# fujii-team/Henbun

Measured on AMD Instinct MI355X. Metric: elbo_samples_per_sec, higher is better.
Workload: dtype f32; 1 GPU; cfg2 SVGP ELBO step: 1-D UnitRBF, N=1e6, M=512 inducing, minibatch 8192 per GPU, diag Normal q(u), diagonal residual, Adam lr 1e-3; global_batch=8192, per_gpu_batch=8192, parallelism=dp1, N=1000000, M=512, dp_exchange=none, dp_ranks=1, contraction=native, tri_pack=False

## Files before the change

### henbun_amd/_lib.py

```python
from __future__ import annotations

import ctypes
import os
from ctypes import c_char_p, c_double, c_int, c_long, c_uint64, c_void_p

_HERE = os.path.dirname(os.path.abspath(__file__))
LIB_PATH = os.path.join(_HERE, "libhenbun_hip.so")


class HipBackendError(RuntimeError):
    """A libhenbun_hip.so entry point returned a non-zero status."""


P, L, I, D, U64 = c_void_p, c_long, c_int, c_double, c_uint64

_SIGS = {
    "hb_version": [],
    "hb_debug_set": [c_char_p, L],
    "hb_debug_clear": [],
    "hb_cholesky_inverse_ws_elems": [L, L, I],
    "hb_cholesky_persistent_shape": [L, L, I],
    "hb_mlp2_sample_supported": [L, L, L, L, L, I],
    "hb_mlp2_sample_ws_elems": [L, L, L],
    "hb_mlp2_sample_fwd_f32": [P, P, P, P, P, I, P, P, L, P, P, P, P, L, L, L, P, P],
    "hb_mlp2_sample_bwd_f32": [P, P, P, P, I, P, P, P, P, P, P, P, P, P, L, L, L, P, P],
    "hb_gram_cholesky_inverse_f32": [I, P, L, P, L, L, L, D, P, P, L, L, P, P, P, I, P],
    "hb_last_error_string": [],
    "hb_device_info": [P, I, P],
    "hb_graph_begin_capture": [P],
    "hb_graph_end_capture": [P, P],
    "hb_graph_launch": [P, P],
    "hb_graph_destroy": [P],
    "hb_rng_init": [P, L, U64, U64, P],
    "hb_rng_randint": [P, L, P, L, L, L, P],
    "hb_sgp_ws_elems": [L, L, L, L, L],
    "hb_sgp_strip_path": [L, L, L, L, L, I],
    "hb_sgp_head_units": [L, L, L, L, L, I, I, I, L],
    "hb_sgp_rider_supported": [L, L, L, L, L, I, I, I, L],
    "hb_sgp_predict_ws_elems": [L, L, L, L, L, I, I, I],
    "hb_sgp_predict_cov_ws_elems": [L, L, L, L, I, I],
    "hb_sgp_stats_ws_elems": [L, L, L, L, I],
    "hb_sgp_select_ws_elems": [L, L, L, I],
    "hb_gram_matvec_chunk": [],
    "hb_gram_matvec_ws_elems": [L, L, L, I],
    "hb_gram_bilinear_grad_ws_elems": [L, L],
    "hb_sgp_kgrad_ws_elems": [L, L, L, L],
    "hb_sgp_wstats_ws_elems": [L, L, L, I],
    "hb_lik_sites_ws_elems": [L],
    "hb_matmul_gauss_units": [L, L, L],
    "hb_matmul_gram_vjp_ok": [L, L, L, L],
    "hb_matmul_gram_vjp_ws_elems": [L, L, L],
    "hb_matmul_gram_vjp_f32": [P, P, P, L, L, L, L, L, L, L, L, L, I, I, P, L, P, L, L, L, P, P, P, P, P],
    "hb_fullrank_one_launch_shape": [L, L],
    "hb_matmul_gauss_f32": [P, L, P, L, P, P, P, P, D, P, P, P, L, L, L, L, P],
    "hb_sgp_rider_begin": [],
    "hb_sgp_rider_pending": [],
    "hb_sgp_rider_flush": [P],
    "hb_sgp_fwd_gauss_f32": [I, I, P, L, P, P, L, P, P, I, P, P, P, L, P, P, P, P, P, L, L, L, L, L, P, P, P, P, D, P, P, P, L, P],
    "hb_ewise_prog_image_bytes": [],
# ... 142 lines not shown
```

### henbun_amd/csrc/sgp.hip

```cpp
#include "common.cuh"
#include "sgp_strip.cuh"
#include "chain.cuh"
#include "chol_persist.cuh"
#include <type_traits>
#include "gemm_tile.cuh"
#include "rng_pairs.cuh"
#include "../../include/henbun_hip.h"

#define SGP_BM 64
#define SGP_BN 128

extern "C" int hb_matmul_f32(const float*, const float*, float*, long, long, long, long, long, long, long, long, long,
                             long, int, int, double, double, const float*, long, int, int, float*, long, void*);
extern "C" int hb_matmul_f64(const double*, const double*, double*, long, long, long, long, long, long, long, long,
                             long, long, int, int, double, double, const double*, long, int, int, double*, long,
                             void*);

template <typename T>
struct SgpArgs {
  const T* x;
  long sx;
  const T* z;
  const T* ell;
  long dl;
// ... 1762 lines not shown
template <typename T>
struct SgpBwdArgs {
  const T* W;
  const T* u;
  const T* A;
  const T* fbar;
  const T* eps;
  const T* v;
  T* Kbar;
  long n, M, P;
  int mode;
  long efast;
  const T* x;
  long sx;
  const T* z;
  const T* ell;
  long dl, d;
  const T* WTf;
  const void* WT3;
  long plane3;
  T* part;
  const T* Af;
  T* Kf;
};

template <typename T>
struct SgpRawB {
  T a, u;
};
template <typename T>
struct SgpRawB4 {
  typedef T VT __attribute__((ext_vector_type(16 / sizeof(T))));
  VT a;
  T u;
};

template <typename T, bool FAST>
__global__ void __launch_bounds__(256) sgp_kbar_kernel(SgpBwdArgs<T> a) {
  typedef TileGemm<T, SGP_BM, SGP_BN, 16, 2, 2> G;
  __shared__ __attribute__((aligned(16))) T lds[G::LDS_ELEMS];
  long e;
  int bx;
  sgp_block(a.efast, e, bx);
  const T* W = a.W + e * a.M * a.M;
  const T* u = a.u + e * a.P * a.M;
  const T* A = a.A + e * a.M * a.n;
// ... 137 lines not shown
  SgpStageZ<D, SGP_STRIP_THREADS> zst;
  SgpStageU<SGP_STRIP_THREADS> ust;
  zst.request(z, M, tid);
  ust.request(a.u + e * a.P * a.M, P, M, tid);
  if (tid < SGP_SN) {
    const int cc = col0 + tid;
    const bool ok = cc < n;
    const int cj = ok ? cc : n - 1;
    cjs[tid] = ok ? sgp_resid_coef<float>(a.eps ? a.eps + e * a.n : nullptr, a.v + e * a.n, fbar, a.n, a.P, a.mode, cj) : 0.f;
#pragma unroll
    for (int p = 0; p < 4; ++p) fbs[p][tid] = (ok && p < P) ? fbar[(long)p * n + cj] : 0.f;
#pragma unroll
    for (int dd = 0; dd < D; ++dd) xss[tid * D + dd] = x[cj * D + dd];
  }
  zst.store(zs, M, tid);
  ust.store(us, P, M, tid);
  __syncthreads();

  if (a.Af) {
    const int nTp = M / 32;
    const long fplane = (long)a.plane3 / a.M * 32 * nS;
    for (int t = w; t < nTp; t += SGP_STRIP_THREADS / 64) {
      float avals[16];
      if (BF3) {
        const __bf16* blk = reinterpret_cast<const __bf16*>(a.Af) + ((((long)e * nTp + t) * nS + bx) << 10) + 8 * lane;
        B8 pl[3][2];
#pragma unroll
        for (int p = 0; p < 3; ++p)
#pragma unroll
          for (int q = 0; q < 2; ++q) pl[p][q] = *reinterpret_cast<const B8*>(blk + p * fplane + 512 * q);
#pragma unroll
        for (int q = 0; q < 2; ++q)
#pragma unroll
          for (int j = 0; j < 8; ++j) avals[8 * q + j] = ((float)pl[2][q][j] + (float)pl[1][q][j]) + (float)pl[0][q][j];
      } else {
        const float* blk = a.Af + ((((long)e * nTp + t) * nS + bx) << 10) + 4 * lane;
        V4 av[4];
#pragma unroll
        for (int v = 0; v < 4; ++v) av[v] = *reinterpret_cast<const V4*>(blk + 256 * v);
#pragma unroll
        for (int v = 0; v < 4; ++v)
#pragma unroll
          for (int s2 = 0; s2 < 4; ++s2) avals[4 * v + s2] = av[v][s2];
      }
      const int k = 32 * t + li;
      float uk[4], usum[4] = {0.f, 0.f, 0.f, 0.f};
#pragma unroll
      for (int p = 0; p < 4; ++p) uk[p] = p < P ? us[p][k] : 0.f;
#pragma unroll
      for (int v = 0; v < 4; ++v) {
        const V4 cj4 = *reinterpret_cast<const V4*>(&cjs[16 * h + 4 * v]);
        V4 fb4[4];
#pragma unroll
        for (int p = 0; p < 4; ++p) fb4[p] = *reinterpret_cast<const V4*>(&fbs[p][16 * h + 4 * v]);
#pragma unroll
        for (int s2 = 0; s2 < 4; ++s2) {
          const int c = 16 * h + 4 * v + s2;
          const float aval = avals[4 * v + s2];
          float val = aval * cj4[s2];
#pragma unroll
          for (int p = 0; p < 4; ++p)
            if (p < P) {
              val += uk[p] * fb4[p][s2];
              usum[p] += fb4[p][s2] * aval;
            }
          if (BF3) {
            const __bf16 b0 = (__bf16)val;
            const float r1 = val - (float)b0;
            const __bf16 b1 = (__bf16)r1;
            K3[0][c][k] = b0, K3[1][c][k] = b1, K3[2][c][k] = (__bf16)(r1 - (float)b1);
          } else {
            Ks[c][k] = val;
          }
        }
      }
#pragma unroll
      for (int p = 0; p < 4; ++p)
        if (p < P) {
          const float tsum = usum[p] + __shfl_xor(usum[p], 32);
          if (h == 0) part[(long)(2 * D + p) * M + k] = tsum;
        }
    }
  } else {
    constexpr int G = BF3 ? 8 : 4;
    const int c = tid & 31, kq = tid >> 5;
    const bool cok = col0 + c < n;
    const int cc = cok ? col0 + c : n - 1;
    const float cj = cjs[c];
    float fb[4];
#pragma unroll
    for (int p = 0; p < 4; ++p) fb[p] = fbs[p][c];
    constexpr int NG = SGP_SM_MAX / (16 * G);
    float av[NG][G];
#pragma unroll
    for (int it = 0; it < NG; ++it)
#pragma unroll
      for (int i = 0; i < G; ++i) {
// ... 65 lines not shown
    float kb[16];
    sgp_acc_t_rows(acc, kb);
    if (col0 + SGP_SN > n) {
#pragma unroll
      for (int i = 0; i < 16; ++i)
        if (col0 + 16 * h + i >= n) kb[i] = 0.f;
    }
    if (a.Kbar) {
      float* kp = Kbar + (long)(32 * tile + li) * n + col0 + 16 * h;
      if ((n & 3) == 0 && col0 + SGP_SN <= n) {
#pragma unroll
        for (int v = 0; v < 4; ++v) {
          V4 q;
#pragma unroll
          for (int s2 = 0; s2 < 4; ++s2) q[s2] = kb[4 * v + s2];
          *reinterpret_cast<V4*>(kp + 4 * v) = q;
        }
      } else {
#pragma unroll
        for (int i = 0; i < 16; ++i)
          if (col0 + 16 * h + i < n) kp[i] = kb[i];
      }
    }
    if (a.Kf && !BF3) sgp_store_frag_rows(a.Kf, kb, e, nT, nS, tile, bx, col0, n, lane);
    if (BF3 && a.Kf)
      sgp_store_frag3_row(reinterpret_cast<__bf16*>(a.Kf), (long)a.plane3 / a.M * 32 * nS, kb, e, nT, nS, tile, bx, lane);
    const int row = 32 * tile + li;
    float zr[D], zacc[D], lacc[D];
#pragma unroll
    for (int dd = 0; dd < D; ++dd) zr[dd] = zs[row * D + dd], zacc[dd] = 0.f, lacc[dd] = 0.f;
#pragma unroll
    for (int i = 0; i < 16; ++i) {
      const int c = 16 * h + i;
      float tt[D], r2 = 0.f;
#pragma unroll
      for (int dd = 0; dd < D; ++dd) {
        tt[dd] = (zr[dd] - xss[c * D + dd]) * col.sc[dd];
        r2 += tt[dd] * tt[dd];
      }
      const float gk = kb[i] * hb_exp2_neg<float>(r2);
#pragma unroll
      for (int dd = 0; dd < D; ++dd) {
        zacc[dd] -= gk * tt[dd];
        lacc[dd] += gk * tt[dd] * tt[dd];
      }
    }
#pragma unroll
// ... 369 lines not shown
__device__ __forceinline__ void sgp_lbar_finish_body(const T* __restrict__ slabs, int S, long E, long M, T* __restrict__ Lbar,
                                                     long vblock, long nvblocks) {
  const long total = E * M * M;
  const long stride = nvblocks * blockDim.x;
  for (long t = vblock * blockDim.x + threadIdx.x; t < total; t += stride) {
    const long rem = t % (M * M);
    const long r = rem / M, c = rem - r * M;
    T acc = T(0);
    if (c <= r) {
      T a0 = T(0), a1 = T(0), a2 = T(0), a3 = T(0);
      int s = 0;
      for (; s + 4 <= S; s += 4) {
        const T v0 = slabs[(long)s * total + t], v1 = slabs[(long)(s + 1) * total + t];
        const T v2 = slabs[(long)(s + 2) * total + t], v3 = slabs[(long)(s + 3) * total + t];
        a0 += v0, a1 += v1, a2 += v2, a3 += v3;
      }
      for (; s < S; ++s) a0 += slabs[(long)s * total + t];
      acc = -((a0 + a1) + (a2 + a3));
    }
    Lbar[t] = acc;
  }
}
template <typename T>
__global__ void __launch_bounds__(256) sgp_lbar_finish_kernel(const T* __restrict__ slabs, int S, long E, long M,
                                                              T* __restrict__ Lbar) {
  sgp_lbar_finish_body<T>(slabs, S, E, M, Lbar, blockIdx.x, gridDim.x);
}

template <typename T>
__device__ __forceinline__ void sgp_strip_finish_body(const T* __restrict__ part, int nS, long M, long d, long dl, long P,
                                                      T* __restrict__ zbar, T* __restrict__ ellbar, T* __restrict__ ubar,
                                                      int bx, int q, long e, T (*red)[64], T* smem) {
  const int nq = (int)(2 * d + P);
  part += e * nS * (long)nq * M;
  if (q >= (int)d && q < 2 * (int)d) {
    if (bx != 0) return;
    T acc = T(0);
    for (int s = threadIdx.x; s < nS; s += 256) acc += part[((long)s * nq + q) * M];
    acc = block_sum(acc, smem);
    if (dl == 1) {
      if (q != (int)d) return;
      T tot = acc;
      for (int qq = (int)d + 1; qq < 2 * (int)d; ++qq) {
        T a2 = T(0);
        for (int s = threadIdx.x; s < nS; s += 256) a2 += part[((long)s * nq + qq) * M];
        tot += block_sum(a2, smem);
// ... 23 lines not shown
  red[sg][ml] = acc;
  __syncthreads();
  if (sg == 0 && m < M) {
    const T tot = (red[0][ml] + red[1][ml]) + (red[2][ml] + red[3][ml]);
    if (q < (int)d)
      zbar[(e * M + m) * d + q] = tot;
    else
      ubar[(e * P + (q - 2 * d)) * M + m] = tot;
  }
}
template <typename T>
__global__ void __launch_bounds__(256) sgp_strip_finish_kernel(const T* __restrict__ part, int nS, long M, long d, long dl,
                                                               long P, T* __restrict__ zbar, T* __restrict__ ellbar,
                                                               T* __restrict__ ubar) {
  __shared__ T red[4][64];
  __shared__ T smem[16];
  sgp_strip_finish_body<T>(part, nS, M, d, dl, P, zbar, ellbar, ubar, (int)blockIdx.x, (int)blockIdx.y, (long)blockIdx.z, red, smem);
}
template <typename T>
__global__ void __launch_bounds__(256) sgp_bwd_finish_kernel(const T* __restrict__ part, int nS, long M, long d, long dl,
                                                             long P, T* __restrict__ zbar, T* __restrict__ ellbar,
                                                             T* __restrict__ ubar, int nb_strip, int nbx,
                                                             const T* __restrict__ slabs, int S, long E,
                                                             T* __restrict__ Lbar) {
  __shared__ T red[4][64];
  __shared__ T smem[16];
  if ((int)blockIdx.x < nb_strip) {
    const int nq = (int)(2 * d + P);
    const int vb = blockIdx.x;
    sgp_strip_finish_body<T>(part, nS, M, d, dl, P, zbar, ellbar, ubar, vb % nbx, (vb / nbx) % nq, (long)(vb / (nbx * nq)), red,
                             smem);
  } else {
    sgp_lbar_finish_body<T>(slabs, S, E, M, Lbar, (long)blockIdx.x - nb_strip, (long)gridDim.x - nb_strip);
  }
}

template <typename T>
__global__ void __launch_bounds__(256) sgp_rowgrad_kernel(const T* __restrict__ x, long sx, const T* __restrict__ z,
                                                          const T* __restrict__ ell, long dl,
                                                          const T* __restrict__ Kbar, const T* __restrict__ A,
                                                          const T* __restrict__ fbar, T* __restrict__ zbar,
                                                          T* __restrict__ ellpart, T* __restrict__ ubar, long n,
                                                          long M, long d, long P) {
  __shared__ T smem[16];
  const long e = blockIdx.y, m = blockIdx.x;
  x += e * sx;
  z += (e * M + m) * d;
  ell += e * dl;
  Kbar += (e * M + m) * n;
  A += (e * M + m) * n;
  fbar += e * P * n;
  const long npass_p = (P + 3) / 4, npass_q = (d + SGP_DREG - 1) / SGP_DREG;
  const long npass = npass_p > npass_q ? npass_p : npass_q;
  for (long pass = 0; pass < npass; ++pass) {
// ... 248 lines not shown
        HB_LAUNCH_CHECK();
        *S_out = (int)S2;
        return 0;
      }
    }
  }
  dim3 grid((unsigned)(pairs * S * E), 1, 1);
  if (prec == HB_PREC_BF16X3)
    hipLaunchKernelGGL(sgp_lbar_frag_kernel<true>, grid, dim3(256), 0, stream, Kf, Af, slabs, (int)M, (int)nS, (int)S, E,
                       (int)pairs);
  else
    hipLaunchKernelGGL(sgp_lbar_frag_kernel<false>, grid, dim3(256), 0, stream, Kf, Af, slabs, (int)M, (int)nS, (int)S, E,
                       (int)pairs);
  HB_LAUNCH_CHECK();
  *S_out = (int)S;
  return 0;
}
static int sgp_lbar_frag_launch(const double*, const double*, double*, long, long, long, long, int, int*, hipStream_t) { return -1; }

template <typename T>
static int sgp_bwd(int kind, int mode, const T* x, long sx, const T* z, const T* ell, long dl, const T* W,
                   const T* Wfrag, int prec, const T* u, const T* eps, const T* A, const T* A_frag, const T* v,
                   const T* fbar, T* Kbar, T* Kbar_frag, T* Lbar, T* ubar, T* zbar, T* ellbar, T* xbar, long E, long n,
                   long M, long d, long P, T* ws, hipStream_t stream) {
  HB_REQUIRE(prec == HB_PREC_NATIVE || prec == HB_PREC_BF16X3, "hb_sgp_bwd: unknown precision %d", prec);
  HB_REQUIRE(kind == HB_KERN_RBF, "hb_sgp_bwd: only the UnitRBF kernel is fused (kind=%d)", kind);
  HB_REQUIRE(mode == HB_SGP_NEGLECTED || mode == HB_SGP_DIAGONAL, "hb_sgp_bwd: unknown mode %d", mode);
  HB_REQUIRE(E >= 0 && n >= 0 && M >= 0 && d >= 1 && P >= 0, "hb_sgp_bwd: bad extents");
  HB_REQUIRE(dl == 1 || dl == d, "hb_sgp_bwd: lengthscales must have 1 or d entries");
  HB_REQUIRE(x && z && ell && W && u && (A || A_frag) && v && fbar && (Kbar || Kbar_frag) && Lbar && ubar && zbar && ellbar && ws,
             "hb_sgp_bwd: NULL pointer");
  HB_REQUIRE((A_frag != nullptr) == (Kbar_frag != nullptr), "hb_sgp_bwd: A_frag and Kbar_frag go together");
  HB_REQUIRE(mode == HB_SGP_NEGLECTED || eps, "hb_sgp_bwd: eps required for the diagonal mode");
  HB_REQUIRE(E <= 65535, "hb_sgp_bwd: too many experts");
  HB_REQUIRE(M * n < 2147483647L && M * M < 2147483647L && n * d < 2147483647L, "hb_sgp_bwd: matrix too large for 32-bit indexing");
  if (E * M == 0) return 0;
  T* ellpart = ws + E * n;
  T* mmws = ellpart + E * M * d;
  const long mmws_elems = 32 * E * M * M;
  const long nS = hb_cdiv(n, SGP_SN);
  const bool strip = sizeof(T) == 4 && Wfrag && !xbar && hb_sgp_strip_path(E, n, M, d, P, prec) &&
                     nS * (2 * d + P) * M * E <= mmws_elems;
  HB_REQUIRE(!A_frag || strip, "hb_sgp_bwd: fragment-major A / Kbar need the column-strip form (see hb_sgp_strip_path)");
  HB_REQUIRE(strip || (A && Kbar), "hb_sgp_bwd: row-major A and Kbar required outside the column-strip form");
  HB_REQUIRE(prec == HB_PREC_NATIVE || strip, "hb_sgp_bwd: bf16x3 needs the column-strip form (fp32, Wfrag, M %% 32 == 0, M <= %d, "
             "d <= %d, P <= 4, no xbar)", SGP_SM_MAX, SGP_DREG);
  if (strip) {
    SgpBwdArgs<T> a;
    a.W = W; a.u = u; a.A = A; a.fbar = fbar; a.eps = eps; a.v = v; a.Kbar = Kbar;
    a.n = n; a.M = M; a.P = P; a.mode = mode;
    a.x = x; a.sx = sx; a.z = z; a.ell = ell; a.dl = dl; a.d = d;
    a.WTf = Wfrag + E * M * M;
    a.WT3 = prec == HB_PREC_BF16X3 ? (const void*)(reinterpret_cast<const unsigned short*>(Wfrag + 2 * E * M * M) + 3 * E * M * M)
                                   : nullptr;
    a.plane3 = E * M * M;
    a.part = mmws;
    a.Af = A_frag; a.Kf = Kbar_frag;
    if (A_frag) a.Kbar = nullptr;
    int rc = sgp_bwd_strip_launch(a, E, nS, stream);
    if (rc) return rc;
    if (A_frag) {
      const long npart = ((nS * (2 * d + P) * M * E + 63) / 64) * 64;
      const long slab_cap = (mmws_elems - npart) / (E * M * M);
      HB_REQUIRE(slab_cap >= 1, "hb_sgp_bwd: workspace too small for the Lbar slabs");
      int S = 0;
      rc = sgp_lbar_frag_launch(Kbar_frag, A_frag, mmws + npart, slab_cap > 32 ? 32 : slab_cap, E, M, nS, prec, &S, stream);
      if (rc) return rc;
      const int nbx = (int)hb_cdiv(M, 64), nb_strip = nbx * (int)(2 * d + P) * (int)E;
      hipLaunchKernelGGL(sgp_bwd_finish_kernel<T>, dim3((unsigned)(nb_strip + hb_stream_grid(E * M * M, 256))), dim3(256), 0, stream,
                         mmws, (int)nS, M, d, dl, P, zbar, ellbar, ubar, nb_strip, nbx, mmws + npart, S, E, Lbar);
      HB_LAUNCH_CHECK();
      return 0;
    }
    hipLaunchKernelGGL(sgp_strip_finish_kernel<T>, dim3((unsigned)hb_cdiv(M, 64), (unsigned)(2 * d + P), (unsigned)E), dim3(256), 0,
                       stream, mmws, (int)nS, M, d, dl, P, zbar, ellbar, ubar);
    HB_LAUNCH_CHECK();
    int rc2 = sgp_matmul(Kbar, A, Lbar, E, M, M, n, n, n, M, M * n, M * n, M * M, 0, 1, -1.0, HB_MM_TRIL_OUT, mmws, mmws_elems,
                         (void*)stream);
    return rc2;
  }
  if (n > 0) {
    SgpBwdArgs<T> a;
    a.W = W; a.u = u; a.A = A; a.fbar = fbar; a.eps = eps; a.v = v; a.Kbar = Kbar;
    a.n = n; a.M = M; a.P = P; a.mode = mode;
    a.x = nullptr; a.sx = 0; a.z = nullptr; a.ell = nullptr; a.dl = 0; a.d = d; a.WTf = nullptr; a.WT3 = nullptr;
    a.plane3 = 0; a.part = nullptr; a.Af = nullptr; a.Kf = nullptr;
    const int nRB = hb_cdiv(M, SGP_BM);
    dim3 grid = sgp_grid(hb_cdiv(n, SGP_BN), sgp_grid_y(E, n, nRB), E, a.efast);
    constexpr long VECH = 16 / sizeof(T);
    const bool vec = P == 1 && M % 16 == 0 && n % VECH == 0 && ((uintptr_t)W % 16 == 0) && ((uintptr_t)A % 16 == 0);
    if (vec)
      hipLaunchKernelGGL((sgp_kbar_kernel<T, true>), grid, dim3(256), 0, stream, a);
    else
      hipLaunchKernelGGL((sgp_kbar_kernel<T, false>), grid, dim3(256), 0, stream, a);
    HB_LAUNCH_CHECK();
  }
  {
    constexpr long VECR = 16 / sizeof(T);
    const bool rvec = d <= SGP_DREG && P <= 4 && n > 0 && n % VECR == 0 && ((uintptr_t)A % 16 == 0) &&
                      ((uintptr_t)Kbar % 16 == 0) && ((uintptr_t)fbar % 16 == 0) && ((uintptr_t)x % 16 == 0) &&
                      (sx * (long)sizeof(T)) % 16 == 0;
    dim3 rgrid((unsigned)M, (unsigned)E);
#define HB_SGP_ROWGRAD(D_)                                                                                           \
  hipLaunchKernelGGL((sgp_rowgrad_vec_kernel<T, D_>), rgrid, dim3(256), 0, stream, x, sx, z, ell, dl, Kbar, A, fbar, \
                     zbar, ellpart, ubar, n, M, P)
    if (rvec && d == 1)
      HB_SGP_ROWGRAD(1);
    else if (rvec && d == 2)
      HB_SGP_ROWGRAD(2);
// ... 21 lines not shown
    if (rc) return rc;
  } else {
    HB_HIP(hb_zero_async(Lbar, sizeof(T) * E * M * M, stream));
  }
  return 0;
}

extern "C" int hb_sgp_bwd_f32(int kind, int mode, const float* x, long sx, const float* z, const float* ell, long dl,
                              const float* W, const float* Wfrag, int prec, const float* u, const float* eps,
                              const float* A, const float* A_frag, const float* v, const float* fbar, float* Kbar,
                              float* Kbar_frag, float* Lbar, float* ubar, float* zbar, float* ellbar, float* xbar, long E,
                              long n, long M, long d, long P, float* ws, void* stream) {
  return sgp_bwd<float>(kind, mode, x, sx, z, ell, dl, W, Wfrag, prec, u, eps, A, A_frag, v, fbar, Kbar, Kbar_frag, Lbar,
                        ubar, zbar, ellbar, xbar, E, n, M, d, P, ws, (hipStream_t)stream);
}
extern "C" int hb_sgp_bwd_f64(int kind, int mode, const double* x, long sx, const double* z, const double* ell,
                              long dl, const double* W, const double* Wfrag, int prec, const double* u, const double* eps,
                              const double* A, const double* A_frag, const double* v, const double* fbar, double* Kbar,
                              double* Kbar_frag, double* Lbar, double* ubar, double* zbar, double* ellbar, double* xbar,
                              long E, long n, long M, long d, long P, double* ws, void* stream) {
  return sgp_bwd<double>(kind, mode, x, sx, z, ell, dl, W, Wfrag, prec, u, eps, A, A_frag, v, fbar, Kbar, Kbar_frag, Lbar,
                         ubar, zbar, ellbar, xbar, E, n, M, d, P, ws, (hipStream_t)stream);
}
```

### henbun_amd/graph.py

```python
from __future__ import annotations

import itertools
import math
from typing import Dict, List, Optional, Sequence, Tuple

import numpy as np

from ._lib import HipBackendError as _HipBackendError

_uid = itertools.count()



class Node:
    __slots__ = ("op", "inputs", "attrs", "outputs", "id")

    def __init__(self, op, inputs, attrs, out_shapes):
        self.op = op
        self.inputs = tuple(inputs)
        self.attrs = attrs
        self.id = next(_uid)
        self.outputs = [Tensor(self, i, tuple(int(d) for d in s)) for i, s in enumerate(out_shapes)]


# ... 805 lines not shown
    axis = axis % nd
    return concat([expand_dims(v, axis) for v in vals], axis)


def matmul(a, b, transpose_a=False, transpose_b=False, bias=None, act="none") -> Tensor:
    a, b = as_tensor(a), as_tensor(b)
    if len(a.shape) < 2 or len(b.shape) < 2:
        raise ValueError("matmul needs rank >= 2 operands")
    m, k = (a.shape[-1], a.shape[-2]) if transpose_a else (a.shape[-2], a.shape[-1])
    k2, n = (b.shape[-1], b.shape[-2]) if transpose_b else (b.shape[-2], b.shape[-1])
    if k != k2:
        raise ValueError("matmul inner dimensions differ: %s x %s" % (a.shape, b.shape))
    la, lb = a.shape[:-2], b.shape[:-2]
    if la and lb and la != lb:
        raise ValueError("matmul batch dimensions differ: %s vs %s" % (la, lb))
    lead = la if la else lb
    ins = (a, b) if bias is None else (a, b, as_tensor(bias))
    return make("matmul", ins, {"ta": bool(transpose_a), "tb": bool(transpose_b), "act": act},
                [tuple(lead) + (m, n)]).outputs[0]


def _matmul_emit(plan, node):
    H = plan.H
    a, b = plan.buf(node.inputs[0]), plan.buf(node.inputs[1])
    bias = plan.buf(node.inputs[2]) if len(node.inputs) > 2 else None
    at = node.attrs
    y = node.outputs[0]
    g = getattr(plan, "_mm_head", {}).get(node.id)
    if g is not None:
        units = H.matmul_gauss_units(y.shape[0], node.inputs[0].shape[1], y.shape[1], plan.dtype)
        ok = (units > 0 and a.stride(1) == 1 and a.stride(0) % 4 == 0 and a.data_ptr() % 16 == 0 and b.stride(1) == 1
              and (bias is None or bias.numel() == y.shape[1]))
        if ok:
            def early(t):
                shp = t.shape
                while t.node.op == "reshape" and t not in plan._buf:
                    t = t.node.inputs[0]
                return plan.buf(t).view(shp)

            post = plan._gll_post.get(g.id)
            head = dict(y=early(g.inputs[0]), var=early(g.inputs[2]), scale=early(g.inputs[3]) if len(g.inputs) > 3 else None,
                        dmu=plan.out(g.outputs[1]), post=post[0] if post else 0.0, fbar=plan.out(post[1]) if post else None,
                        part=plan.scratch((3 * units,)), units=units)
            plan._gll_fused[g.id] = (head["part"], units)
            plan.pin_side_reads([g.inputs[0], g.inputs[2]] + list(g.inputs[3:4]))
            plan.steps.append(lambda: H.matmul_gauss(a, b, bias, head))
# ... 113 lines not shown
    if n.op in ("cholesky", "trinv"):
        return True
    if n.op == "sgp_grad":
        return t.index == 0
    if n.op == "matutil":
        return n.attrs["mode"] == 2 or (n.attrs["mode"] == 0 and n.attrs["upper"] == 0)
    if n.op == "stop_gradient":
        return _known_lower(n.inputs[0])
    return False


def band_part(x, num_lower, num_upper):
    x = as_tensor(x)
    if int(num_lower) < 0 and int(num_upper) == 0 and _known_lower(x):
        return x
    return matutil(x, 0, num_lower, num_upper)


def add_eye(x, alpha):
    return matutil(x, 1, alpha=alpha)


def _matutil_emit(plan, node):
    if node.id in plan._fused_matutil:
        return
    H = plan.H
    x, out = plan.buf(node.inputs[0]), plan.out(node.outputs[0])
    a = node.attrs
    plan.steps.append(lambda: H.matutil(x, a["mode"], a["lower"], a["upper"], a["alpha"], out=out))


def _matutil_vjp(node, gs):
    g = gs[0]
    if g is None:
        return [None]
    a = node.attrs
    if a["mode"] == 0:
        return [matutil(g, 0, a["lower"], a["upper"])]
    if a["mode"] == 1:
        return [g]
    if a["mode"] == 2:
        return [matutil(g, 2)]
    if a["mode"] == 4:
        return [matutil(matutil(g, 3), 2)]
    return [matutil(g, 3)]


# ... 644 lines not shown
                plan.step_labels[id(cell["step"])] = "cholesky+sgp"
                plan.step_riders[id(cell["step"])] = node
                plan.note(ep, node, True)
                return
            plan.note(ep, node, False, "an operand is produced after the factorisation has been launched")
    plan.steps.append(step)
    plan.chain_kind[id(step)] = "tail"


def _sgp_vjp(node, gs):
    gf = gs[0]
    if gf is None:
        return [None] * len(node.inputs)
    if any(g is not None for g in gs[1:3]):
        raise NotImplementedError("gradients through the A / v outputs of sgp_samples")
    x, z, ell, L, W, u = node.inputs[:6]
    f, A, v, eps = node.outputs
    n = make("sgp_grad", (x, z, ell, W, u, eps, A, v, gf), {"mode": node.attrs["mode"]},
             [L.shape, u.shape, z.shape, ell.shape, x.shape])
    Lb, ub, zb, lb, xb = n.outputs
    return [xb, zb, lb, Lb, None, ub] + [None] * (len(node.inputs) - 6)


def _sgp_grad_emit(plan, node):
    H = plan.H
    x, z, ell, W, u, eps, A, v, gf = (plan.buf(t) for t in node.inputs)
    Lb, ub, zb, lb, xb = (plan.out(t) for t in node.outputs)
    mode = SGP_MODES[node.attrs["mode"]]
    need_x = plan.needed(node.outputs[4])
    if need_x and len(node.inputs[1].shape) > 2 and len(node.inputs[0].shape) == 2:
        raise NotImplementedError("gradient w.r.t. an x shared by several experts")
    xbuf = xb.reshape((-1,) + tuple(xb.shape[-2:])) if need_x else None
    wfrag, bf3 = plan._wfrag.get(_through_stop_gradient(node.inputs[3]), (None, False))
    bf3 = bf3 and not need_x and node.inputs[0].shape[-1] <= 4 and node.inputs[4].shape[-2] <= 4
    prec = H.PREC_BF16X3 if bf3 else H.PREC_NATIVE
    a_frag, fprec = plan._afrag.get(node.inputs[6], (None, None))
    if a_frag is not None:
        prec = fprec
    kbar_frag = plan.scratch((a_frag.numel(),)) if a_frag is not None else None
    Kbar = plan.scratch(A.shape) if a_frag is None else None
    plan.steps.append(lambda: H.sgp_bwd(x, z, ell, W, u, eps, A, v, gf, mode=mode, need_xbar=need_x,
                                        out=(Kbar, Lb, ub, zb, lb, xbuf), wfrag=wfrag, prec=prec, a_frag=a_frag,
                                        kbar_frag=kbar_frag))


defop("sgp", _sgp_emit, _sgp_vjp)
defop("sgp_grad", _sgp_grad_emit, None)

SGP_PREDICT_MODES = {"neglected": 0, "diagonal": 1, "fullrank": 2}
SGP_PREDICT_S = {"diag": 0, "tril": 1}

# ... 462 lines not shown
        self.trail_version = None
        self.chain_kind: Dict[int, str] = {}
        self.chain_members: Dict[int, list] = {}
        self._chains_fused = False
        self.step_labels = {}
        self.step_nodes = {}
        self.noise_inputs: Dict[Tensor, object] = {}
        self._injected: Dict[Tensor, bool] = {}
        self._leaf_resolver = leaf_resolver
        order = topo_order(self.outputs)
        self._order_pos = {n.id: i for i, n in enumerate(order)}
        self._order = order
        self._needed = set()
        for n in order:
            for t in n.inputs:
                self._needed.add(t)
        for t in self.outputs:
            self._needed.add(t)
        self._extra_copies = []
        self._fused_trinv = set()
        self._wfrag: Dict[Tensor, object] = {}
        self._afrag: Dict[Tensor, object] = {}
        self._fused_matutil = set()
        self._fused_concat = set()
        self._lazy_cols: Dict[Tensor, object] = {}
        for t, b in (binds or []):
            self._prebind(t, b)
        if prologue:
            prologue(self)
        from ._settings import settings as _st

        fuse = bool(getattr(_st.runtime, "fuse_elementwise", True))
        consumers0 = {}
        for n in order:
            for t in n.inputs:
                consumers0.setdefault(t, []).append(n)
        self._gll_post: Dict[int, tuple] = {}
        self._absorbed = set()
        if fuse:
            outs_set = set(self.outputs)
            for n in order:
                if n.op == "gauss_ll":
                    post = _gauss_ll_post(n, consumers0, outs_set)
                    if post is not None and not any(m.id in self._absorbed for m in post[2]):
                        self._gll_post[n.id] = post
                        self._absorbed.update(m.id for m in post[2])
# ... 672 lines not shown
```

### henbun_amd/hip_ops.py

```python
from __future__ import annotations

import ctypes
from ctypes import c_double, c_int, c_long, c_void_p

import numpy as np
import torch

from . import _lib

EW = dict(
    NEG=1, EXP=2, LOG=3, SQRT=4, SQUARE=5, ABS=6, SIGN=7, SIGMOID=8, RELU=9, SOFTPLUS=10, TANH=11,
    RECIP=12, RSQRT=13, STEP=14, AFFINE=15, CLIP=16, CLIPMASK=17, LGAMMA=18, POWC=19, LOG1P=20,
    COPY=21, DIGAMMA=22,
    ADD=32, SUB=33, MUL=34, DIV=35, MAX=36, MIN=37, POW=38, GT=39, GE=40, LT=41, LE=42, EQ=43,
    SIGMOID_GRAD=44, TANH_GRAD=45, RELU_GRAD=46, SOFTPLUS_GRAD=47, CLIP_GRAD=48,
    WHERE=64, FMA=65, GAUSS_LOGPDF=66,
    GAUSS_LOGPDF_GRAD=80,
)
RED_SUM, RED_MAX = 0, 1
KERN_RBF, KERN_CSYM_RBF, KERN_SQDIST = 0, 1, 2
KERN_KBAR_SYMMETRIC = 256
EW_PROG_SUM = 256
MM_LOWER_OUT = 1
MM_TRIL_OUT = 2
# ... 1286 lines not shown
            prec=PREC_NATIVE, a_frag=None, kbar_frag=None):
    E, n, M, d, P, sx = _sgp_dims(x, z, u)
    dev, dt = x.device, x.dtype
    dl = ell.numel() // E
    if out is None:
        Kbar = _empty_like(A) if a_frag is None else None
        Lbar = _empty_like(W)
        ubar = _empty_like(u)
        zbar = _empty_like(z)
        ellbar = _empty_like(ell)
        xbar = _empty((E, n, d), dtype=dt, device=dev) if need_xbar else None
    else:
        Kbar, Lbar, ubar, zbar, ellbar, xbar = out
    wse = _lib.lib().raw("hb_sgp_ws_elems")(E, n, M, d, P)
    ws = workspace(dt, dev, wse)
    if a_frag is not None and kbar_frag is None:
        kbar_frag = _empty(a_frag.numel(), dtype=dt, device=dev)
    _lib.lib().call("hb_sgp_bwd" + _suf(x), KERN_RBF, mode, _p(x), sx, _p(z), _p(ell), dl, _p(W), _p(wfrag), int(prec), _p(u), _p(eps),
                    _p(A) if a_frag is None else None, _p(a_frag), _p(v), _p(fbar), _p(Kbar) if a_frag is None else None,
                    _p(kbar_frag), _p(Lbar), _p(ubar), _p(zbar), _p(ellbar), _p(xbar), E, n, M, d, P, _p(ws), stream())
    return Lbar, ubar, zbar, ellbar, xbar


def adam_step(theta, g, m, v, t, lr=1e-3, b1=0.9, b2=0.999, eps=1e-8, gscale=1.0, tick=True, info=None, dpflag=None,
              fail=None):
    assert t.dtype == torch.int64
    n_info = 0
    if info is not None:
        assert info.dtype == torch.int32 and info.is_contiguous()
        n_info = info.numel()
    if fail is not None:
        assert fail.dtype == torch.int64 and fail.numel() == 2
    if dpflag is not None:
        assert dpflag.dtype == theta.dtype and dpflag.numel() == 1
    _lib.lib().call("hb_adam_step" + _suf(theta), _p(theta), _p(g), _p(m), _p(v), theta.numel(), float(lr), float(b1),
                    float(b2), float(eps), float(gscale), _p(t), int(bool(tick)), _p(info) if n_info else None, n_info,
                    _p(dpflag) if dpflag is not None else None, _p(fail) if fail is not None else None, stream())


def allreduce_sum(flat, comm_handle):
    _chk(flat)
    _lib.lib().call("hb_allreduce_sum" + _suf(flat), _p(flat), flat.numel(), comm_handle, stream())


def dp_pack(tail, objective, info):
    assert tail.numel() == 2
# ... 34 lines not shown
```

### include/henbun_hip.h

```cpp
#ifndef HENBUN_HIP_H
#define HENBUN_HIP_H

#include <stdint.h>

#ifdef __cplusplus
extern "C" {
#endif

#define HB_ABI_VERSION 2

int hb_version(void);
const char* hb_last_error_string(void);
int hb_debug_set(const char* key, long value);
int hb_debug_clear(void);
int hb_device_info(char* buf, int buflen, int* cu_count);

int hb_graph_begin_capture(void* stream);
int hb_graph_end_capture(void* stream, void** exec_out);
int hb_graph_launch(void* exec, void* stream);
int hb_graph_destroy(void* exec);

enum {
  HB_EW_NEG = 1, HB_EW_EXP, HB_EW_LOG, HB_EW_SQRT, HB_EW_SQUARE, HB_EW_ABS, HB_EW_SIGN,
  HB_EW_SIGMOID, HB_EW_RELU, HB_EW_SOFTPLUS, HB_EW_TANH, HB_EW_RECIP, HB_EW_RSQRT,
// ... 319 lines not shown
int hb_gram_bilinear_grad_f64(int kind, const double* x, const double* ell, long dl, const double* A, const double* B,
                              const double* w, double* g, long N, long d, long S, double* ws, void* stream);
long hb_sgp_select_ws_elems(long N, long M, long d, int dtype_bytes);
int hb_sgp_select_f32(int kind, const float* X, const float* ell, long dl, long N, long M, long d, double threshold, long* idx,
                      float* pivots, long* count, double* trace, float* ws, void* stream);
int hb_sgp_select_f64(int kind, const double* X, const double* ell, long dl, long N, long M, long d, double threshold,
                      long* idx, double* pivots, long* count, double* trace, double* ws, void* stream);
long hb_sgp_kgrad_ws_elems(long N, long M, long d, long P);
int hb_sgp_kgrad_f32(int kind, const float* X, const float* Y, const double* z, const double* ell, long dl, const double* Q,
                     const double* R, double* zbar, double* ellbar, long N, long M, long d, long P, double* ws, void* stream);
int hb_sgp_kgrad_f64(int kind, const double* X, const double* Y, const double* z, const double* ell, long dl, const double* Q,
                     const double* R, double* zbar, double* ellbar, long N, long M, long d, long P, double* ws, void* stream);
int hb_sgp_wkgrad_f32(int kind, const float* X, const double* w, const double* r, const double* z, const double* ell, long dl,
                      const double* Q, const double* R, double* zbar, double* ellbar, long N, long M, long d, double* ws,
                      void* stream);
int hb_sgp_wkgrad_f64(int kind, const double* X, const double* w, const double* r, const double* z, const double* ell, long dl,
                      const double* Q, const double* R, double* zbar, double* ellbar, long N, long M, long d, double* ws,
                      void* stream);
int hb_sgp_bwd_f32(int kind, int mode, const float* x, long sx, const float* z, const float* ell,
                   long dl, const float* W, const float* Wfrag, int prec, const float* u, const float* eps,
                   const float* A, const float* A_frag, const float* v, const float* fbar, float* Kbar,
                   float* Kbar_frag, float* Lbar, float* ubar, float* zbar, float* ellbar, float* xbar,
                   long E, long n, long M, long d, long P, float* ws, void* stream);
int hb_sgp_bwd_f64(int kind, int mode, const double* x, long sx, const double* z, const double* ell,
                   long dl, const double* W, const double* Wfrag, int prec, const double* u,
                   const double* eps, const double* A, const double* A_frag, const double* v,
                   const double* fbar, double* Kbar, double* Kbar_frag, double* Lbar, double* ubar,
                   double* zbar, double* ellbar, double* xbar, long E, long n, long M, long d, long P,
                   double* ws, void* stream);

int hb_adam_step_f32(float* theta, const float* g, float* m, float* v, long n, double lr, double b1,
                     double b2, double eps, double gscale, long* t, int tick, const int* info,
                     long n_info, const float* dpflag, long* fail, void* stream);
int hb_adam_step_f64(double* theta, const double* g, double* m, double* v, long n, double lr,
                     double b1, double b2, double eps, double gscale, long* t, int tick,
                     const int* info, long n_info, const double* dpflag, long* fail, void* stream);

int hb_side_push_gather_draw_f32(int narr, const float* const* srcs, const long* rows, float* const* dsts, long nsrc,
                                 uint64_t* state, long nlanes, long lo, long hi, long* idx_out, const long* perm,
                                 long n, int* err, void* stream);
int hb_side_push_diag_fwd_f32(const float* mu, const float* s, const float* u_in, uint64_t* rng, long rng_lanes,
                              float* u_out, float* x, float* kl, long n, long L, long ld_mu, long ld_s, float* ws,
                              void* stream);
int hb_side_push_diag_bwd_f32(const float* s, const float* u, const float* x, const float* xbar, const float* klbar,
                              float* mubar, float* sbar, long n, long L, long ld_s, long ld_out, void* stream);
int hb_side_pending(void);
// ... 25 lines not shown
```

Baseline: 42.14 million samples/s.

## Fold Cholesky VJP's first product into sparse-GP backward via Abar fragments

The Lbar computation and the following L^T tril(Lbar) product plus Phisym are folded into the SGP backward. The strip kernel now writes Abar (Kbar scaled by A) in fragment layout, and the slab reduction multiplies against that. A new finish body then writes the symmetrised Phi directly in 32x32 tile pairs. This removes a separate MxM matmul, a tril pass and a Phisym pass from the backward, at the cost of a new graph pattern matcher and a different fold kernel.

```diff
diff --git a/henbun_amd/_lib.py b/henbun_amd/_lib.py
--- a/henbun_amd/_lib.py
+++ b/henbun_amd/_lib.py
@@ -35,6 +35,8 @@
     "hb_rng_randint": [P, L, P, L, L, L, P],
     "hb_sgp_ws_elems": [L, L, L, L, L],
     "hb_sgp_strip_path": [L, L, L, L, L, I],
+    "hb_sgp_bwd_phi_supported": [L, L, L, L, L],
+    "hb_sgp_bwd_phi_f32": [I, I, P, L, P, P, L, P, P, P, P, P, P, P, P, P, P, P, P, L, L, L, L, L, P, P],
     "hb_sgp_head_units": [L, L, L, L, L, I, I, I, L],
     "hb_sgp_rider_supported": [L, L, L, L, L, I, I, I, L],
     "hb_sgp_predict_ws_elems": [L, L, L, L, L, I, I, I],
diff --git a/henbun_amd/csrc/sgp.hip b/henbun_amd/csrc/sgp.hip
--- a/henbun_amd/csrc/sgp.hip
+++ b/henbun_amd/csrc/sgp.hip
@@ -1808,6 +1808,7 @@
   T* part;
   const T* Af;
   T* Kf;
+  T* Abf;
 };
 
 template <typename T>
@@ -1991,6 +1992,7 @@
     const long fplane = (long)a.plane3 / a.M * 32 * nS;
     for (int t = w; t < nTp; t += SGP_STRIP_THREADS / 64) {
       float avals[16];
+      long abf_off = 0;
       if (BF3) {
         const __bf16* blk = reinterpret_cast<const __bf16*>(a.Af) + ((((long)e * nTp + t) * nS + bx) << 10) + 8 * lane;
         B8 pl[3][2];
@@ -2003,7 +2005,8 @@
 #pragma unroll
           for (int j = 0; j < 8; ++j) avals[8 * q + j] = ((float)pl[2][q][j] + (float)pl[1][q][j]) + (float)pl[0][q][j];
       } else {
-        const float* blk = a.Af + ((((long)e * nTp + t) * nS + bx) << 10) + 4 * lane;
+        abf_off = ((((long)e * nTp + t) * nS + bx) << 10) + 4 * lane;
+        const float* blk = a.Af + abf_off;
         V4 av[4];
 #pragma unroll
         for (int v = 0; v < 4; ++v) av[v] = *reinterpret_cast<const V4*>(blk + 256 * v);
@@ -2022,6 +2025,7 @@
         V4 fb4[4];
 #pragma unroll
         for (int p = 0; p < 4; ++p) fb4[p] = *reinterpret_cast<const V4*>(&fbs[p][16 * h + 4 * v]);
+        V4 ab4;
 #pragma unroll
         for (int s2 = 0; s2 < 4; ++s2) {
           const int c = 16 * h + 4 * v + s2;
@@ -2040,8 +2044,10 @@
             K3[0][c][k] = b0, K3[1][c][k] = b1, K3[2][c][k] = (__bf16)(r1 - (float)b1);
           } else {
             Ks[c][k] = val;
+            ab4[s2] = val;
           }
         }
+        if (!BF3 && a.Abf) *reinterpret_cast<V4*>(a.Abf + abf_off + 256 * v) = ab4;
       }
 #pragma unroll
       for (int p = 0; p < 4; ++p)
@@ -2153,7 +2159,7 @@
           if (col0 + 16 * h + i < n) kp[i] = kb[i];
       }
     }
-    if (a.Kf && !BF3) sgp_store_frag_rows(a.Kf, kb, e, nT, nS, tile, bx, col0, n, lane);
+    if (a.Kf && !BF3 && !a.Abf) sgp_store_frag_rows(a.Kf, kb, e, nT, nS, tile, bx, col0, n, lane);
     if (BF3 && a.Kf)
       sgp_store_frag3_row(reinterpret_cast<__bf16*>(a.Kf), (long)a.plane3 / a.M * 32 * nS, kb, e, nT, nS, tile, bx, lane);
     const int row = 32 * tile + li;
@@ -2569,6 +2575,69 @@
   }
 }
 template <typename T>
+__device__ __forceinline__ void sgp_phi_finish_body(const T* __restrict__ slabs, int S, long E, long M, T* __restrict__ Phi,
+                                                    long vblock, long nvblocks, T (*tile)[33]) {
+  const long total = E * M * M;
+  const int nT = (int)(M / 32), pairs = nT * (nT + 1) / 2;
+  const long units = E * pairs * 2;
+  for (long unit = vblock; unit < units; unit += nvblocks) {
+    const long e = unit / (2 * pairs);
+    const int rest = (int)(unit - e * 2 * pairs), pair = rest >> 1, r0 = 16 * (rest & 1);
+    int ti = (int)((sqrtf(8.f * (float)pair + 1.f) - 1.f) * 0.5f);
+    while (ti * (ti + 1) / 2 > pair) --ti;
+    while ((ti + 1) * (ti + 2) / 2 <= pair) ++ti;
+    const int tj = pair - ti * (ti + 1) / 2;
+    const bool diag = ti == tj;
+    long t[2];
+    T a[2][4], val[2];
+#pragma unroll
+    for (int k = 0; k < 2; ++k) {
+      const int idx = threadIdx.x + 256 * k, r = idx >> 5, c = idx & 31;
+      t[k] = (e * M + 32 * ti + r0 + r) * M + 32 * tj + c;
+#pragma unroll
+      for (int q = 0; q < 4; ++q) a[k][q] = T(0);
+    }
+    int s = 0;
+    for (; s + 4 <= S; s += 4) {
+      T v[2][4];
+#pragma unroll
+      for (int k = 0; k < 2; ++k)
+#pragma unroll
+        for (int q = 0; q < 4; ++q) v[k][q] = slabs[(long)(s + q) * total + t[k]];
+#pragma unroll
+      for (int k = 0; k < 2; ++k)
+#pragma unroll
+        for (int q = 0; q < 4; ++q) a[k][q] += v[k][q];
+    }
+    {
+      T v[2][3];
+#pragma unroll
+      for (int k = 0; k < 2; ++k)
+#pragma unroll
+        for (int q = 0; q < 3; ++q) v[k][q] = s + q < S ? slabs[(long)(s + q) * total + t[k]] : T(0);
+#pragma unroll
+      for (int k = 0; k < 2; ++k)
+#pragma unroll
+        for (int q = 0; q < 3; ++q)
+          if (s + q < S) a[k][0] += v[k][q];
+    }
+#pragma unroll
+    for (int k = 0; k < 2; ++k) {
+      const int idx = threadIdx.x + 256 * k, r = idx >> 5, c = idx & 31;
+      val[k] = T(0.5) * -((a[k][0] + a[k][1]) + (a[k][2] + a[k][3]));
+      tile[r][c] = val[k];
+      if (!diag || c <= r0 + r) Phi[t[k]] = val[k];
+    }
+    __syncthreads();
+#pragma unroll
+    for (int k = 0; k < 2; ++k) {
+      const int idx = threadIdx.x + 256 * k, c = idx >> 4, r = idx & 15;
+      if (!diag || c < r0 + r) Phi[(e * M + 32 * tj + c) * M + 32 * ti + r0 + r] = tile[r][c];
+    }
+    __syncthreads();
+  }
+}
+template <typename T>
 __global__ void __launch_bounds__(256) sgp_lbar_finish_kernel(const T* __restrict__ slabs, int S, long E, long M,
                                                               T* __restrict__ Lbar) {
   sgp_lbar_finish_body<T>(slabs, S, E, M, Lbar, blockIdx.x, gridDim.x);
@@ -2638,14 +2707,17 @@
                                                              long P, T* __restrict__ zbar, T* __restrict__ ellbar,
                                                              T* __restrict__ ubar, int nb_strip, int nbx,
                                                              const T* __restrict__ slabs, int S, long E,
-                                                             T* __restrict__ Lbar) {
+                                                             T* __restrict__ Lbar, int phi) {
   __shared__ T red[4][64];
   __shared__ T smem[16];
+  __shared__ T tile[32][33];
   if ((int)blockIdx.x < nb_strip) {
     const int nq = (int)(2 * d + P);
     const int vb = blockIdx.x;
     sgp_strip_finish_body<T>(part, nS, M, d, dl, P, zbar, ellbar, ubar, vb % nbx, (vb / nbx) % nq, (long)(vb / (nbx * nq)), red,
                              smem);
+  } else if (phi) {
+    sgp_phi_finish_body<T>(slabs, S, E, M, Lbar, (long)blockIdx.x - nb_strip, (long)gridDim.x - nb_strip, tile);
   } else {
     sgp_lbar_finish_body<T>(slabs, S, E, M, Lbar, (long)blockIdx.x - nb_strip, (long)gridDim.x - nb_strip);
   }
@@ -2940,7 +3012,7 @@
 static int sgp_bwd(int kind, int mode, const T* x, long sx, const T* z, const T* ell, long dl, const T* W,
                    const T* Wfrag, int prec, const T* u, const T* eps, const T* A, const T* A_frag, const T* v,
                    const T* fbar, T* Kbar, T* Kbar_frag, T* Lbar, T* ubar, T* zbar, T* ellbar, T* xbar, long E, long n,
-                   long M, long d, long P, T* ws, hipStream_t stream) {
+                   long M, long d, long P, T* ws, hipStream_t stream, T* Abar_frag = nullptr) {
   HB_REQUIRE(prec == HB_PREC_NATIVE || prec == HB_PREC_BF16X3, "hb_sgp_bwd: unknown precision %d", prec);
   HB_REQUIRE(kind == HB_KERN_RBF, "hb_sgp_bwd: only the UnitRBF kernel is fused (kind=%d)", kind);
   HB_REQUIRE(mode == HB_SGP_NEGLECTED || mode == HB_SGP_DIAGONAL, "hb_sgp_bwd: unknown mode %d", mode);
@@ -2963,6 +3035,8 @@
   HB_REQUIRE(strip || (A && Kbar), "hb_sgp_bwd: row-major A and Kbar required outside the column-strip form");
   HB_REQUIRE(prec == HB_PREC_NATIVE || strip, "hb_sgp_bwd: bf16x3 needs the column-strip form (fp32, Wfrag, M %% 32 == 0, M <= %d, "
              "d <= %d, P <= 4, no xbar)", SGP_SM_MAX, SGP_DREG);
+  HB_REQUIRE(!Abar_frag || (strip && A_frag && prec == HB_PREC_NATIVE),
+             "hb_sgp_bwd_phi: needs the column-strip form in native precision with a fragment-major A (see hb_sgp_bwd_phi_supported)");
   if (strip) {
     SgpBwdArgs<T> a;
     a.W = W; a.u = u; a.A = A; a.fbar = fbar; a.eps = eps; a.v = v; a.Kbar = Kbar;
@@ -2973,7 +3047,7 @@
                                    : nullptr;
     a.plane3 = E * M * M;
     a.part = mmws;
-    a.Af = A_frag; a.Kf = Kbar_frag;
+    a.Af = A_frag; a.Kf = Kbar_frag; a.Abf = Abar_frag;
     if (A_frag) a.Kbar = nullptr;
     int rc = sgp_bwd_strip_launch(a, E, nS, stream);
     if (rc) return rc;
@@ -2982,11 +3056,13 @@
       const long slab_cap = (mmws_elems - npart) / (E * M * M);
       HB_REQUIRE(slab_cap >= 1, "hb_sgp_bwd: workspace too small for the Lbar slabs");
       int S = 0;
-      rc = sgp_lbar_frag_launch(Kbar_frag, A_frag, mmws + npart, slab_cap > 32 ? 32 : slab_cap, E, M, nS, prec, &S, stream);
+      rc = sgp_lbar_frag_launch(Abar_frag ? Abar_frag : Kbar_frag, A_frag, mmws + npart, slab_cap > 32 ? 32 : slab_cap, E, M, nS, prec, &S, stream);
       if (rc) return rc;
       const int nbx = (int)hb_cdiv(M, 64), nb_strip = nbx * (int)(2 * d + P) * (int)E;
-      hipLaunchKernelGGL(sgp_bwd_finish_kernel<T>, dim3((unsigned)(nb_strip + hb_stream_grid(E * M * M, 256))), dim3(256), 0, stream,
-                         mmws, (int)nS, M, d, dl, P, zbar, ellbar, ubar, nb_strip, nbx, mmws + npart, S, E, Lbar);
+      const long nTl = M / 32, phi_units = E * nTl * (nTl + 1);
+      const long nb_fold = Abar_frag ? (phi_units < 2048 ? phi_units : 2048) : (long)hb_stream_grid(E * M * M, 256);
+      hipLaunchKernelGGL(sgp_bwd_finish_kernel<T>, dim3((unsigned)(nb_strip + nb_fold)), dim3(256), 0, stream,
+                         mmws, (int)nS, M, d, dl, P, zbar, ellbar, ubar, nb_strip, nbx, mmws + npart, S, E, Lbar, Abar_frag ? 1 : 0);
       HB_LAUNCH_CHECK();
       return 0;
     }
@@ -3002,7 +3078,7 @@
     a.W = W; a.u = u; a.A = A; a.fbar = fbar; a.eps = eps; a.v = v; a.Kbar = Kbar;
     a.n = n; a.M = M; a.P = P; a.mode = mode;
     a.x = nullptr; a.sx = 0; a.z = nullptr; a.ell = nullptr; a.dl = 0; a.d = d; a.WTf = nullptr; a.WT3 = nullptr;
-    a.plane3 = 0; a.part = nullptr; a.Af = nullptr; a.Kf = nullptr;
+    a.plane3 = 0; a.part = nullptr; a.Af = nullptr; a.Kf = nullptr; a.Abf = nullptr;
     const int nRB = hb_cdiv(M, SGP_BM);
     dim3 grid = sgp_grid(hb_cdiv(n, SGP_BN), sgp_grid_y(E, n, nRB), E, a.efast);
     constexpr long VECH = 16 / sizeof(T);
@@ -3070,3 +3146,18 @@
   return sgp_bwd<double>(kind, mode, x, sx, z, ell, dl, W, Wfrag, prec, u, eps, A, A_frag, v, fbar, Kbar, Kbar_frag, Lbar,
                          ubar, zbar, ellbar, xbar, E, n, M, d, P, ws, (hipStream_t)stream);
 }
+
+extern "C" int hb_sgp_bwd_phi_supported(long E, long n, long M, long d, long P) {
+  if (hb_debug_get("sgp_phi_direct", 1) == 0) return 0;
+  return hb_sgp_strip_path(E, n, M, d, P, HB_PREC_NATIVE);
+}
+
+extern "C" int hb_sgp_bwd_phi_f32(int kind, int mode, const float* x, long sx, const float* z, const float* ell, long dl,
+                                  const float* W, const float* Wfrag, const float* u, const float* eps, const float* A_frag,
+                                  const float* v, const float* fbar, float* Abar_frag, float* Phi, float* ubar, float* zbar,
+                                  float* ellbar, long E, long n, long M, long d, long P, float* ws, void* stream) {
+  HB_REQUIRE(Wfrag && A_frag && Abar_frag && Phi, "hb_sgp_bwd_phi: NULL pointer");
+  HB_REQUIRE(hb_sgp_strip_path(E, n, M, d, P, HB_PREC_NATIVE), "hb_sgp_bwd_phi: shape outside the column-strip form (see hb_sgp_strip_path)");
+  return sgp_bwd<float>(kind, mode, x, sx, z, ell, dl, W, Wfrag, HB_PREC_NATIVE, u, eps, nullptr, A_frag, v, fbar, nullptr,
+                        Abar_frag, Phi, ubar, zbar, ellbar, nullptr, E, n, M, d, P, ws, (hipStream_t)stream, Abar_frag);
+}
diff --git a/henbun_amd/graph.py b/henbun_amd/graph.py
--- a/henbun_amd/graph.py
+++ b/henbun_amd/graph.py
@@ -851,6 +851,8 @@
 
 def _matmul_emit(plan, node):
     H = plan.H
+    if node.id in plan._phi_direct:
+        return
     a, b = plan.buf(node.inputs[0]), plan.buf(node.inputs[1])
     bias = plan.buf(node.inputs[2]) if len(node.inputs) > 2 else None
     at = node.attrs
@@ -1010,7 +1012,7 @@
 
 
 def _matutil_emit(plan, node):
-    if node.id in plan._fused_matutil:
+    if node.id in plan._fused_matutil or node.id in plan._phi_direct:
         return
     H = plan.H
     x, out = plan.buf(node.inputs[0]), plan.out(node.outputs[0])
@@ -1701,11 +1703,69 @@
     return [xb, zb, lb, Lb, None, ub] + [None] * (len(node.inputs) - 6)
 
 
+PHI_DIRECT = "Cholesky VJP's first product folded into the sparse-GP backward (hb_sgp_bwd_phi)"
+
+
+def _phi_direct_match(plan, node, a_frag, prec, need_x):
+    H = plan.H
+    if a_frag is None:
+        return None, "A is exchanged row-major (no column-strip form, or A / xbar is read elsewhere)"
+    if plan.dtype != plan.torch.float32 or prec != H.PREC_NATIVE or need_x:
+        return None, "needs fp32 operands in native precision"
+    Lb, skipped = node.outputs[0], []
+
+    def private(t):
+        return len(plan._consumers.get(t, [])) == 1 and t not in plan.outputs and t not in plan._bind
+
+    if not private(Lb):
+        return None, "Lbar is a plan output, or has a reader besides the Cholesky VJP's product"
+    c = plan._consumers[Lb][0]
+    t = Lb
+    if c.op == "matutil" and c.attrs["mode"] == 0 and c.attrs["lower"] < 0 and c.attrs["upper"] == 0:
+        t = c.outputs[0]
+        if not private(t):
+            return None, "tril(Lbar) is a plan output, or has a second reader"
+        skipped.append(c.id)
+        c = plan._consumers[t][0]
+    at = c.attrs
+    if not (c.op == "matmul" and len(c.inputs) == 2 and c.inputs[1] is t and c.inputs[0] is not t and at["ta"] and not at["tb"]
+            and at["act"] == "none" and not at.get("actgrad")):
+        return None, "Lbar does not feed the product L^T tril(Lbar)"
+    L, Q = c.inputs[0], c.outputs[0]
+    Wsrc, fwd = _through_stop_gradient(node.inputs[3]), node.inputs[6].node
+    if not (Wsrc.node.op == "trinv" and Wsrc.node.inputs[0] is L and fwd.op == "sgp" and fwd.inputs[3] is L
+            and _through_stop_gradient(fwd.inputs[4]) is Wsrc):
+        return None, "the product's left operand is not the factor L whose inverse whitened the draw"
+    if not private(Q) or c.id in plan._colsum_of or c.id in getattr(plan, "_mm_head", {}):
+        return None, "L^T tril(Lbar) is a plan output, or has a reader besides Phisym"
+    mu = plan._consumers[Q][0]
+    if not (mu.op == "matutil" and mu.attrs["mode"] == 4):
+        return None, "L^T tril(Lbar) is not followed by Phisym (matutil mode 4)"
+    zsh, xsh = node.inputs[1].shape, node.inputs[0].shape
+    E, M, n, d, P = int(np.prod(zsh[:-2])) if len(zsh) > 2 else 1, zsh[-2], xsh[-2], xsh[-1], node.inputs[4].shape[-2]
+    if not H.sgp_bwd_phi_supported(E, n, M, d, P):
+        return None, "shape outside the column-strip form, or switched off (hb_debug_set sgp_phi_direct 0)"
+    return (mu, skipped + [c.id, mu.id]), None
+
+
 def _sgp_grad_emit(plan, node):
     H = plan.H
     x, z, ell, W, u, eps, A, v, gf = (plan.buf(t) for t in node.inputs)
+    mode = SGP_MODES[node.attrs["mode"]]
+    if plan.needed(node.outputs[0]):
+        a_frag, fprec = plan._afrag.get(node.inputs[6], (None, None))
+        hit, why = _phi_direct_match(plan, node, a_frag, fprec, plan.needed(node.outputs[4]))
+        plan.note(PHI_DIRECT, node, hit is not None, why or "")
+        if hit is not None:
+            mu, skipped = hit
+            plan._phi_direct.update(skipped)
+            wfrag = plan._wfrag[_through_stop_gradient(node.inputs[3])][0]
+            outs = (plan.out(mu.outputs[0]),) + tuple(plan.out(t) for t in node.outputs[1:4])
+            abar_frag = plan.scratch((a_frag.numel(),))
+            plan.steps.append(lambda: H.sgp_bwd_phi(x, z, ell, W, u, eps, v, gf, wfrag, a_frag, mode=mode, out=outs,
+                                                    abar_frag=abar_frag))
+            return
     Lb, ub, zb, lb, xb = (plan.out(t) for t in node.outputs)
-    mode = SGP_MODES[node.attrs["mode"]]
     need_x = plan.needed(node.outputs[4])
     if need_x and len(node.inputs[1].shape) > 2 and len(node.inputs[0].shape) == 2:
         raise NotImplementedError("gradient w.r.t. an x shared by several experts")
@@ -2214,6 +2274,7 @@
         self._wfrag: Dict[Tensor, object] = {}
         self._afrag: Dict[Tensor, object] = {}
         self._fused_matutil = set()
+        self._phi_direct = set()
         self._fused_concat = set()
         self._lazy_cols: Dict[Tensor, object] = {}
         for t, b in (binds or []):
diff --git a/henbun_amd/hip_ops.py b/henbun_amd/hip_ops.py
--- a/henbun_amd/hip_ops.py
+++ b/henbun_amd/hip_ops.py
@@ -1332,6 +1332,28 @@
     return Lbar, ubar, zbar, ellbar, xbar
 
 
+def sgp_bwd_phi_supported(E, n, M, d, P):
+    return bool(_lib.lib().raw("hb_sgp_bwd_phi_supported")(E, n, M, d, P))
+
+
+def sgp_bwd_phi(x, z, ell, W, u, eps, v, fbar, wfrag, a_frag, mode=SGP_DIAGONAL, out=None, abar_frag=None):
+    E, n, M, d, P, sx = _sgp_dims(x, z, u)
+    dev, dt = x.device, x.dtype
+    assert dt == torch.float32 and wfrag is not None and a_frag is not None
+    dl = ell.numel() // E
+    if out is None:
+        Phi, ubar, zbar, ellbar = _empty_like(W), _empty_like(u), _empty_like(z), _empty_like(ell)
+    else:
+        Phi, ubar, zbar, ellbar = out
+    ws = workspace(dt, dev, _lib.lib().raw("hb_sgp_ws_elems")(E, n, M, d, P))
+    if abar_frag is None:
+        abar_frag = _empty(a_frag.numel(), dtype=dt, device=dev)
+    assert abar_frag.numel() >= sgp_frag_elems(E, n, M)
+    _lib.lib().call("hb_sgp_bwd_phi_f32", KERN_RBF, mode, _p(x), sx, _p(z), _p(ell), dl, _p(W), _p(wfrag), _p(u), _p(eps), _p(a_frag),
+                    _p(v), _p(fbar), _p(abar_frag), _p(Phi), _p(ubar), _p(zbar), _p(ellbar), E, n, M, d, P, _p(ws), stream())
+    return Phi, ubar, zbar, ellbar
+
+
 def adam_step(theta, g, m, v, t, lr=1e-3, b1=0.9, b2=0.999, eps=1e-8, gscale=1.0, tick=True, info=None, dpflag=None,
               fail=None):
     assert t.dtype == torch.int64
diff --git a/include/henbun_hip.h b/include/henbun_hip.h
--- a/include/henbun_hip.h
+++ b/include/henbun_hip.h
@@ -365,6 +365,11 @@
                    const float* A, const float* A_frag, const float* v, const float* fbar, float* Kbar,
                    float* Kbar_frag, float* Lbar, float* ubar, float* zbar, float* ellbar, float* xbar,
                    long E, long n, long M, long d, long P, float* ws, void* stream);
+int hb_sgp_bwd_phi_supported(long E, long n, long M, long d, long P);
+int hb_sgp_bwd_phi_f32(int kind, int mode, const float* x, long sx, const float* z, const float* ell, long dl,
+                       const float* W, const float* Wfrag, const float* u, const float* eps, const float* A_frag,
+                       const float* v, const float* fbar, float* Abar_frag, float* Phi, float* ubar, float* zbar,
+                       float* ellbar, long E, long n, long M, long d, long P, float* ws, void* stream);
 int hb_sgp_bwd_f64(int kind, int mode, const double* x, long sx, const double* z, const double* ell,
                    long dl, const double* W, const double* Wfrag, int prec, const double* u,
                    const double* eps, const double* A, const double* A_frag, const double* v,
```

Result: faster. 43.26 million samples/s, median of 6 (+2.7%).
